# osheraz/IsaacGymInsertion

Measured on AMD Instinct MI355X. Metric: PPO update steps/sec (4096 envs x 32 horizon), higher is better.
Workload: dtype f32; 1 GPU; teacher PPO update, MLP actor-critic 404,501 params, 4096 envs x 32 horizon per GPU, 8 mini-epochs x 8 minibatches of 16384 (BASELINE configs[1]); envs_per_gpu=4096, horizon=32, optimizer_steps_per_update=64, parallelism=dp1, grad_allreduce=none

## Files before the change

### isaacgyminsertion_amd/csrc/fwd12.h

```cpp
#pragma once
#include "policy_fwd.h"

namespace igi {

struct Fwd12Args {
  const float* priv; int ldp;
  float* xcat; int ldx;
  int M, obs;
  const float *eW1, *eb1, *eW2, *eb2, *eW3, *eb3;
  const float* w1p;
  const float* tb1; long long ac_block;
  float* e1; int lde1;
  float* e2; int lde2;
  float* h1; int ldh; long long sH;
};

constexpr int F12_NW = 8;
constexpr int F12_NS = 3;
constexpr int F12_THREADS = 64 * (F12_NW + 4);
constexpr int F12_RING = F12_NW * F12_NS * PF_CH;
constexpr int F12_PRIV = 2 * PF_IMG;
constexpr int F12_Q = 8 * PF_IMG;
constexpr int F12_LDS_FLOATS = PF_P + F12_Q + F12_RING + 2 * F12_PRIV + 2 * PF_IMG + PF_IMG + 8 * 128 + 32 * 8;
static_assert(F12_LDS_FLOATS * 4 <= 160 * 1024, "LDS budget");

template <int NIMG>
__device__ __forceinline__ void f12_store_images(const float* __restrict__ img, float* __restrict__ g, long long ldg, int rows_ok, int st) {
#pragma unroll
  for (int i = 0; i < NIMG; ++i) {
    const int rem = st, r = rem >> 3, slot = rem & 7;
    const int p = slot ^ ((r >> 1) & 7);
    const f32x4 v = *reinterpret_cast<const f32x4*>(img + i * PF_IMG + r * 32 + slot * 4);
    if (r < rows_ok) *reinterpret_cast<f32x4*>(g + (long long)r * ldg + 32 * i + 4 * p) = v;
  }
}

__device__ __forceinline__ void f12_barrier() {
  asm volatile("s_waitcnt lgkmcnt(0)" ::: "memory");
  __builtin_amdgcn_s_barrier();
  asm volatile("" ::: "memory");
}

__global__ __launch_bounds__(F12_THREADS) void k_fwd12(const Fwd12Args a) {
  extern __shared__ __attribute__((aligned(1024))) float smem[];
  float* P = smem;
  float* Q = P + PF_P;
  float* ring0 = Q + F12_Q;
  float* privb = ring0 + F12_RING;
  float* xsb = privb + 2 * F12_PRIV;
  float* X = xsb + 2 * PF_IMG;
  float* w3s = X + PF_IMG;
  float* lat = w3s + 8 * 128;
  const int tid = threadIdx.x, lane = tid & 63, wave = __builtin_amdgcn_readfirstlane(tid >> 6);
  const bool compute = wave < F12_NW;
  const int dw = compute ? wave : wave - F12_NW;
  const int nblocks = (a.M + PF_ROWS - 1) / PF_ROWS;
  PfWave w;
  w.ring = ring0 + dw * (F12_NS * PF_CH);
  w.lane = lane; w.wave = wave; w.l31 = lane & 31; w.h = lane >> 5;
  pf_img_bases(w.l31, w.h, w.ib);
  w.aoff = w.l31 * 32; w.asw = (w.l31 >> 1) & 7;
  w.boff = w.l31 * 16; w.bsw = (w.l31 >> 2) & 3;
  const int st = tid - 64 * F12_NW;

  auto issue_inputs = [&](int b, int buf) {
    const int m0 = b * PF_ROWS;
#pragma unroll
    for (int q = 0; q < 2; ++q) {
      const int piece = dw + 4 * q, k = piece >> 2, i = piece & 3;
      const int m = 8 * i + (lane >> 3);
      const int row = min(m0 + m, a.M - 1);
      dma16(a.priv + (long long)row * a.ldp + k * 32 + 4 * ((lane & 7) ^ ((m >> 1) & 7)), privb + buf * F12_PRIV + k * PF_IMG + 256 * i);
    }
    const int xr = 8 * dw + (lane >> 3);
    dma16(a.xcat + (long long)min(m0 + xr, a.M - 1) * a.ldx + 4 * (lane & 7), xsb + buf * PF_IMG + 256 * dw);
  };

  const int c31 = 32 * (wave & 7) + w.l31;
  float be1[1] = {a.eb1[c31]};
  float be2[1] = {a.eb2[c31 & 127]};
  float bt1[4][1];
#pragma unroll
  for (int u = 0; u < 4; ++u) bt1[u][0] = a.tb1[(u >> 1) * a.ac_block + 256 * (u & 1) + c31];
  const float b3 = a.eb3[(tid >> 5) & 7];
  int b = blockIdx.x;
  if (!compute && b < nblocks) issue_inputs(b, 0);
  for (int e = tid; e < 8 * 128; e += F12_THREADS) w3s[e] = a.eW3[e];
  asm volatile("s_waitcnt vmcnt(0)" ::: "memory");
  f12_barrier();

  int it = 0;
  for (; b < nblocks; b += gridDim.x, ++it) {
    const int m0 = b * PF_ROWS;
    const int rows_ok = min(PF_ROWS, a.M - m0);
    const bool more = b + (int)gridDim.x < nblocks;
    if (compute) pf_layer<64, 256, 1, F12_NW, F12_NS>(w, privb + (it & 1) * F12_PRIV, a.eW1, 64, be1, P);
    f12_barrier();
    if (compute) pf_layer<256, 128, 1, F12_NW, F12_NS>(w, P, a.eW2, 256, be2, Q);
    else f12_store_images<8>(P, a.e1 + (long long)m0 * a.lde1, a.lde1, rows_ok, st);
    f12_barrier();
    if (tid < 256) {
      const int row = tid & 31, out = tid >> 5;
      const float* xr = Q + row * 32;
      const float* wr = w3s + out * 128;
      const int sw = (row >> 1) & 7;
      float acc = 0.f;
#pragma unroll 4
      for (int c8 = 0; c8 < 128; c8 += 8) {
        const float* im = xr + (c8 >> 5) * PF_IMG;
        const int p0 = (c8 & 31) >> 2;
        const f32x4 x0 = *reinterpret_cast<const f32x4*>(im + ((p0 ^ sw) << 2)), x1 = *reinterpret_cast<const f32x4*>(im + (((p0 + 1) ^ sw) << 2));
        const f32x4 u0 = *reinterpret_cast<const f32x4*>(wr + c8), u1 = *reinterpret_cast<const f32x4*>(wr + c8 + 4);
#pragma unroll
        for (int j = 0; j < 4; ++j) {
          acc = fmaf(x0[j], u0[j], acc);
          acc = fmaf(x1[j], u1[j], acc);
        }
      }
      lat[row * 8 + out] = fast_tanh(acc + b3);
    } else if (!compute) {
      f12_store_images<4>(Q, a.e2 + (long long)m0 * a.lde2, a.lde2, rows_ok, st);
    }
    f12_barrier();
    if (!compute) {
      const int xrow = st >> 3, xc = 4 * (st & 7), sw = (xrow >> 1) & 7;
      f32x4 v = *reinterpret_cast<const f32x4*>(xsb + (it & 1) * PF_IMG + xrow * 32 + xc);
#pragma unroll
      for (int q = 0; q < 4; ++q) {
        const int c = xc + q;
        if (c >= a.obs && c < a.obs + 8) v[q] = lat[xrow * 8 + (c - a.obs)];
      }
      *reinterpret_cast<f32x4*>(X + xrow * 32 + (((xc >> 2) ^ sw) << 2)) = v;
      const int j = st & 7;
      if (xrow < rows_ok) a.xcat[(long long)(m0 + xrow) * a.ldx + a.obs + j] = lat[xrow * 8 + j];
    }
    f12_barrier();
    if (!compute && more) issue_inputs(b + gridDim.x, (it + 1) & 1);
#pragma unroll
    for (int u = 0; u < 4; ++u) {
      if (compute) {
        pf_layer<32, 256, 1, F12_NW, F12_NS>(w, X, a.w1p + (long long)((u >> 1) * 512 + 256 * (u & 1)) * 32, 32, bt1[u], (u & 1) ? Q : P);
      } else if (u > 0) {
        const int v = u - 1;
        f12_store_images<8>((v & 1) ? Q : P, a.h1 + (v >> 1) * a.sH + (long long)m0 * a.ldh + 256 * (v & 1), a.ldh, rows_ok, st);
      }
      if (u == 3 && !compute && more) {
        asm volatile("s_waitcnt vmcnt(24)" ::: "memory");
      }
      f12_barrier();
    }
    if (!compute) f12_store_images<8>(Q, a.h1 + a.sH + (long long)m0 * a.ldh + 256, a.ldh, rows_ok, st);
  }
}

static inline bool fwd12_supported(int K1, int N1, int N2, int N3, int obs, int xld, int u0) {
  return K1 == 64 && N1 == 256 && N2 == 128 && N3 == 8 && obs >= 1 && obs + 8 <= 32 && xld == 32 && u0 == 512;
}

static hipError_t fwd12_forward(const Fwd12Args& a, hipStream_t s) {
  if (a.M < 1 || !aligned16(a.priv) || !aligned16(a.xcat) || (a.ldp & 3) || a.ldp < 64 || a.ldx != 32 || !aligned16(a.eW1) ||
      !aligned16(a.eW2) || !aligned16(a.eW3) || !aligned16(a.w1p) || !aligned16(a.e1) || !aligned16(a.e2) || !aligned16(a.h1) || (a.lde1 & 3) ||
      (a.lde2 & 3) || (a.ldh & 3) || (a.sH & 3) || a.lde1 < 256 || a.lde2 < 128 || a.ldh < 512)
    return hipErrorInvalidValue;
  static bool attr = false;
  if (!attr) {
    hipError_t e = hipFuncSetAttribute((const void*)k_fwd12, hipFuncAttributeMaxDynamicSharedMemorySize, (int)(sizeof(float) * F12_LDS_FLOATS));
    if (e != hipSuccess) return e;
    attr = true;
  }
  const int nblocks = (a.M + PF_ROWS - 1) / PF_ROWS;
  const int grid = nblocks < 256 ? nblocks : 256;
  const double fl = 2.0 * a.M * (64.0 * 256 + 256.0 * 128 + 128.0 * 8 + 2.0 * (a.obs + 8) * 512.0);
  const double by = 4.0 * a.M * (64.0 + a.obs + 256 + 128 + 8 + 1024) + 4.0 * (64.0 * 256 + 256.0 * 128 + 2 * 512.0 * 32);
  ProfScope ps(PC_FWD12, s, fl, by);
  IGI_LAUNCH(k_fwd12, dim3(grid), dim3(F12_THREADS), sizeof(float) * F12_LDS_FLOATS, s, a);
  return hipGetLastError();
}

}
```

Measured before the change: 40.16 updates/s.

## Software-pipeline the actor/critic first-layer units with deferred epilogues and inline MFMA

Replaces the generic pf_layer calls for the four 32->256 actor/critic first-layer units with a hand-written per-unit MFMA path. It prefetches the next unit's weights while computing the current one. Half of the compute waves defer their tanh epilogue by one phase, and the last unit's epilogue spills into the next block's iteration, so the stores to h1 are split into halves and overlapped with the next block's encoder layers. An extra LDS region E is added and the xcat double buffer is dropped to pay for it. The goal is to hide weight-load latency and the store tail, at the cost of much more intricate cross-iteration state and barrier ordering.

Result: no change. 40.10 updates/s (median of 2 runs) (-0.1%).

```diff
diff --git a/isaacgyminsertion_amd/csrc/fwd12.h b/isaacgyminsertion_amd/csrc/fwd12.h
--- a/isaacgyminsertion_amd/csrc/fwd12.h
+++ b/isaacgyminsertion_amd/csrc/fwd12.h
@@ -21,7 +21,8 @@
 constexpr int F12_RING = F12_NW * F12_NS * PF_CH;
 constexpr int F12_PRIV = 2 * PF_IMG;
 constexpr int F12_Q = 8 * PF_IMG;
-constexpr int F12_LDS_FLOATS = PF_P + F12_Q + F12_RING + 2 * F12_PRIV + 2 * PF_IMG + PF_IMG + 8 * 128 + 32 * 8;
+constexpr int F12_E = 4 * PF_IMG;
+constexpr int F12_LDS_FLOATS = PF_P + F12_Q + F12_E + F12_RING + 2 * F12_PRIV + PF_IMG + PF_IMG + 8 * 128 + 32 * 8;
 static_assert(F12_LDS_FLOATS * 4 <= 160 * 1024, "LDS budget");
 
 template <int NIMG>
@@ -41,18 +42,71 @@
   asm volatile("" ::: "memory");
 }
 
+template <int U>
+__device__ __forceinline__ void f12_unit_request(const PfWave& w, const float* __restrict__ w1p, unsigned (&goff)[2]) {
+  const float* Wt = w1p + (long long)((U >> 1) * 512 + 256 * (U & 1) + 32 * w.wave) * 32;
+#pragma unroll
+  for (int c = 0; c < 2; ++c) {
+    float* dst = w.ring + ((2 * U + c) % F12_NS) * PF_CH;
+    const char* base = reinterpret_cast<const char*>(uniform_ptr(Wt + 16 * c));
+#pragma unroll
+    for (int i = 0; i < 2; ++i) {
+      asm volatile("" : "+v"(goff[i]));
+      dma16(reinterpret_cast<const float*>(base + goff[i]), dst + 256 * i);
+    }
+  }
+}
+
+template <int U>
+__device__ __forceinline__ void f12_unit_mma(const PfWave& w, const float* __restrict__ X, const float* __restrict__ w1p, unsigned (&goff)[2],
+                                             f32x16& acc) {
+  asm volatile("s_waitcnt vmcnt(0)" ::: "memory");
+  f32x4 fa[2][2], fb[2][2];
+#pragma unroll
+  for (int c = 0; c < 2; ++c) {
+    const float* ch = w.ring + ((2 * U + c) % F12_NS) * PF_CH;
+#pragma unroll
+    for (int g = 0; g < 2; ++g) {
+      const int g8 = 2 * c + g;
+      fa[c][g] = *reinterpret_cast<const f32x4*>(X + w.aoff + (((2 * g8 + w.h) ^ w.asw) << 2));
+      fb[c][g] = *reinterpret_cast<const f32x4*>(ch + w.boff + (((2 * g + w.h) ^ w.bsw) << 2));
+    }
+  }
+  if constexpr (U < 3) {
+    asm volatile("s_waitcnt lgkmcnt(0)" ::: "memory");
+    f12_unit_request<(U < 3 ? U + 1 : 0)>(w, w1p, goff);
+  }
+#pragma unroll
+  for (int r = 0; r < 16; ++r) acc[r] = 0.f;
+  __builtin_amdgcn_sched_barrier(0);
+#pragma unroll
+  for (int c = 0; c < 2; ++c)
+#pragma unroll
+    for (int g = 0; g < 2; ++g)
+#pragma unroll
+      for (int q = 0; q < 4; ++q) acc = __builtin_amdgcn_mfma_f32_32x32x2f32(fa[c][g][q], fb[c][g][q], acc, 0, 0, 0);
+  __builtin_amdgcn_sched_barrier(0);
+}
+
+__device__ __forceinline__ void f12_unit_epilogue(const PfWave& w, const f32x16& acc, float bias, float* __restrict__ img) {
+#pragma unroll
+  for (int r = 0; r < 16; ++r) img[w.ib[(r >> 1) & 3] + ((r & 3) + 8 * (r >> 2)) * 32] = fast_tanh(acc[r] + bias);
+}
+
 __global__ __launch_bounds__(F12_THREADS) void k_fwd12(const Fwd12Args a) {
   extern __shared__ __attribute__((aligned(1024))) float smem[];
   float* P = smem;
   float* Q = P + PF_P;
-  float* ring0 = Q + F12_Q;
+  float* E = Q + F12_Q;
+  float* ring0 = E + F12_E;
   float* privb = ring0 + F12_RING;
   float* xsb = privb + 2 * F12_PRIV;
-  float* X = xsb + 2 * PF_IMG;
+  float* X = xsb + PF_IMG;
   float* w3s = X + PF_IMG;
   float* lat = w3s + 8 * 128;
   const int tid = threadIdx.x, lane = tid & 63, wave = __builtin_amdgcn_readfirstlane(tid >> 6);
   const bool compute = wave < F12_NW;
+  const bool late = wave >= F12_NW / 2;
   const int dw = compute ? wave : wave - F12_NW;
   const int nblocks = (a.M + PF_ROWS - 1) / PF_ROWS;
   PfWave w;
@@ -62,6 +116,12 @@
   w.aoff = w.l31 * 32; w.asw = (w.l31 >> 1) & 7;
   w.boff = w.l31 * 16; w.bsw = (w.l31 >> 2) & 3;
   const int st = tid - 64 * F12_NW;
+  unsigned goff[2];
+#pragma unroll
+  for (int i = 0; i < 2; ++i) {
+    const int r = 16 * i + (lane >> 2), p = (lane & 3) ^ ((r >> 2) & 3);
+    goff[i] = 4u * ((unsigned)r * 32u + 4u * (unsigned)p);
+  }
 
   auto issue_inputs = [&](int b, int buf) {
     const int m0 = b * PF_ROWS;
@@ -73,15 +133,18 @@
       dma16(a.priv + (long long)row * a.ldp + k * 32 + 4 * ((lane & 7) ^ ((m >> 1) & 7)), privb + buf * F12_PRIV + k * PF_IMG + 256 * i);
     }
     const int xr = 8 * dw + (lane >> 3);
-    dma16(a.xcat + (long long)min(m0 + xr, a.M - 1) * a.ldx + 4 * (lane & 7), xsb + buf * PF_IMG + 256 * dw);
+    dma16(a.xcat + (long long)min(m0 + xr, a.M - 1) * a.ldx + 4 * (lane & 7), xsb + 256 * dw);
+  };
+  auto store_half = [&](const float* img, int u, int hi, int m0, int rows_ok) {
+    f12_store_images<4>(img, a.h1 + (u >> 1) * a.sH + (long long)m0 * a.ldh + 256 * (u & 1) + 128 * hi, a.ldh, rows_ok, st);
   };
 
   const int c31 = 32 * (wave & 7) + w.l31;
   float be1[1] = {a.eb1[c31]};
   float be2[1] = {a.eb2[c31 & 127]};
-  float bt1[4][1];
-#pragma unroll
-  for (int u = 0; u < 4; ++u) bt1[u][0] = a.tb1[(u >> 1) * a.ac_block + 256 * (u & 1) + c31];
+  float bt1[4];
+#pragma unroll
+  for (int u = 0; u < 4; ++u) bt1[u] = a.tb1[(u >> 1) * a.ac_block + 256 * (u & 1) + c31];
   const float b3 = a.eb3[(tid >> 5) & 7];
   int b = blockIdx.x;
   if (!compute && b < nblocks) issue_inputs(b, 0);
@@ -89,15 +152,30 @@
   asm volatile("s_waitcnt vmcnt(0)" ::: "memory");
   f12_barrier();
 
-  int it = 0;
+  f32x16 held;
+#pragma unroll
+  for (int r = 0; r < 16; ++r) held[r] = 0.f;
+  int it = 0, m0 = 0, rows_ok = 0;
   for (; b < nblocks; b += gridDim.x, ++it) {
-    const int m0 = b * PF_ROWS;
-    const int rows_ok = min(PF_ROWS, a.M - m0);
+    const int pm0 = m0;
+    m0 = b * PF_ROWS;
+    rows_ok = min(PF_ROWS, a.M - m0);
     const bool more = b + (int)gridDim.x < nblocks;
-    if (compute) pf_layer<64, 256, 1, F12_NW, F12_NS>(w, privb + (it & 1) * F12_PRIV, a.eW1, 64, be1, P);
-    f12_barrier();
-    if (compute) pf_layer<256, 128, 1, F12_NW, F12_NS>(w, P, a.eW2, 256, be2, Q);
-    else f12_store_images<8>(P, a.e1 + (long long)m0 * a.lde1, a.lde1, rows_ok, st);
+    if (compute) {
+      if (late && it > 0) f12_unit_epilogue(w, held, bt1[3], Q + wave * PF_IMG);
+      pf_layer<64, 256, 1, F12_NW, F12_NS>(w, privb + (it & 1) * F12_PRIV, a.eW1, 64, be1, P);
+    } else if (it > 0) {
+      store_half(Q, 3, 0, pm0, PF_ROWS);
+      store_half(E, 2, 1, pm0, PF_ROWS);
+    }
+    f12_barrier();
+    if (compute) {
+      pf_layer<256, 128, 1, F12_NW, F12_NS>(w, P, a.eW2, 256, be2, Q);
+      f12_unit_request<0>(w, a.w1p, goff);
+    } else {
+      f12_store_images<8>(P, a.e1 + (long long)m0 * a.lde1, a.lde1, rows_ok, st);
+      if (it > 0) store_half(Q + 4 * PF_IMG, 3, 1, pm0, PF_ROWS);
+    }
     f12_barrier();
     if (tid < 256) {
       const int row = tid & 31, out = tid >> 5;
@@ -118,13 +196,11 @@
         }
       }
       lat[row * 8 + out] = fast_tanh(acc + b3);
-    } else if (!compute) {
-      f12_store_images<4>(Q, a.e2 + (long long)m0 * a.lde2, a.lde2, rows_ok, st);
     }
     f12_barrier();
     if (!compute) {
       const int xrow = st >> 3, xc = 4 * (st & 7), sw = (xrow >> 1) & 7;
-      f32x4 v = *reinterpret_cast<const f32x4*>(xsb + (it & 1) * PF_IMG + xrow * 32 + xc);
+      f32x4 v = *reinterpret_cast<const f32x4*>(xsb + xrow * 32 + xc);
 #pragma unroll
       for (int q = 0; q < 4; ++q) {
         const int c = xc + q;
@@ -136,20 +212,40 @@
     }
     f12_barrier();
     if (!compute && more) issue_inputs(b + gridDim.x, (it + 1) & 1);
-#pragma unroll
-    for (int u = 0; u < 4; ++u) {
+    auto phase = [&](auto u_c) {
+      constexpr int U = decltype(u_c)::value;
+      float* lo = (U & 1) ? Q : P;
       if (compute) {
-        pf_layer<32, 256, 1, F12_NW, F12_NS>(w, X, a.w1p + (long long)((u >> 1) * 512 + 256 * (u & 1)) * 32, 32, bt1[u], (u & 1) ? Q : P);
-      } else if (u > 0) {
-        const int v = u - 1;
-        f12_store_images<8>((v & 1) ? Q : P, a.h1 + (v >> 1) * a.sH + (long long)m0 * a.ldh + 256 * (v & 1), a.ldh, rows_ok, st);
-      }
-      if (u == 3 && !compute && more) {
-        asm volatile("s_waitcnt vmcnt(24)" ::: "memory");
+        if (!late) {
+          f32x16 acc;
+          f12_unit_mma<U>(w, X, a.w1p, goff, acc);
+          f12_unit_epilogue(w, acc, bt1[U], lo + wave * PF_IMG);
+        } else {
+          float* hi = U == 3 ? E + (wave - F12_NW / 2) * PF_IMG : ((U & 1) ? P : Q) + wave * PF_IMG;
+          if constexpr (U > 0) f12_unit_epilogue(w, held, bt1[U > 0 ? U - 1 : 0], hi);
+          f12_unit_mma<U>(w, X, a.w1p, goff, held);
+        }
+      } else {
+        if constexpr (U == 0) f12_store_images<4>(Q, a.e2 + (long long)m0 * a.lde2, a.lde2, rows_ok, st);
+        if constexpr (U >= 2) store_half(((U & 1) ? Q : P) + 4 * PF_IMG, U - 2, 1, m0, rows_ok);
+        if constexpr (U >= 1) store_half((U & 1) ? P : Q, U - 1, 0, m0, rows_ok);
+        if constexpr (U == 3) {
+          if (more) asm volatile("s_waitcnt vmcnt(24)" ::: "memory");
+        }
       }
       f12_barrier();
-    }
-    if (!compute) f12_store_images<8>(Q, a.h1 + a.sH + (long long)m0 * a.ldh + 256, a.ldh, rows_ok, st);
+    };
+    pf_for<0, 4>(phase);
+  }
+  if (it > 0) {
+    if (compute) {
+      if (late) f12_unit_epilogue(w, held, bt1[3], Q + wave * PF_IMG);
+    } else {
+      store_half(Q, 3, 0, m0, rows_ok);
+      store_half(E, 2, 1, m0, rows_ok);
+    }
+    f12_barrier();
+    if (!compute) store_half(Q + 4 * PF_IMG, 3, 1, m0, rows_ok);
   }
 }
 
```
